# lusinlu/Video-Generation-for-Human-Avatars

Measured on AMD Instinct MI355X. Metric: LTX-2B LoRA train-step samples/sec (latent-tokens/sec = samples/sec x 1792), higher is better.
Workload: dtype bf16; 1 GPU; LTX-Video 2B LoRA(r=16, attn2 q/k/v/out) + caption_projection train step, 49f 512x512 -> latent 7x16x16 (N=1792), 1xMI355X per rank; lora_rank=16, model=LTX-Video-2B (28 layers, D 2048, 32x64 heads), global_batch=8, micro_batch_per_gpu=8, seq_len=1792, text_len=256, grad_accum=16, parallelism=dp1, attn2_padding_blocks=skipped, exact

## Files before the change

### include/ltx_hip.h

```cpp
#ifndef LTX_HIP_H_
#define LTX_HIP_H_

#include <stdint.h>

#ifdef __cplusplus
extern "C" {
#endif

enum {
  LTX_OK = 0,
  LTX_ERR_BAD_ARG = 1000,
  LTX_ERR_UNSUPPORTED = 1001,
};

enum {
  LTX_EPI_STORE = 0,
  LTX_EPI_GELU = 1,
  LTX_EPI_GATED_RESIDUAL = 2,
  LTX_EPI_LORA = 3,
  LTX_EPI_LORA_RESIDUAL = 4,
  LTX_EPI_GELU_BWD = 5,
  LTX_EPI_ACCUM = 6,
  LTX_EPI_LORA_DGRAD_ACCUM = 7,
  LTX_EPI_STORE_ROWDOT = 8,
// ... 4 lines not shown
int ltx_device_info(int* gfx_arch, int* num_cus);

int ltx_patchify_bf16(const void* latents, void* tokens, int64_t B, int64_t C, int64_t F,
                      int64_t H, int64_t W, void* stream);
int ltx_unpatchify_bf16(const void* tokens, void* latents, int64_t B, int64_t C, int64_t F,
                        int64_t H, int64_t W, void* stream);
int ltx_latent_coords(int64_t* coords, int64_t B, int64_t F, int64_t H, int64_t W, void* stream);

int ltx_rf_noise_velocity(const void* tokens, const void* noise, const float* t, void* x_t,
                          void* v_target, int64_t B, int64_t NC, void* stream);
int ltx_rf_noise_velocity_f32(const void* tokens, int tokens_f32, const void* noise, int noise_f32,
                              const float* t, float* x_t, float* v_target, int64_t B, int64_t NC,
                              void* stream);
int ltx_condition_lerp(const void* tokens, const void* ref, const void* pose, void* out,
                       int64_t B, int64_t C, int64_t F, int64_t H, int64_t W, void* stream);
int ltx_rf_prepare_tokens(const void* latents, const void* ref, const void* pose,
                          const void* noise, const float* t, void* x_t, void* model_in,
                          void* v_target, int64_t B, int64_t C, int64_t F, int64_t H, int64_t W,
                          void* stream);

int ltx_rmsnorm_modulate_fwd(const void* x, const void* shift, const void* onep, int64_t ld_mod,
                             void* y, float* rstd, int64_t M, int64_t D, int64_t rows_per_batch,
                             float eps, void* stream);
int ltx_rmsnorm_modulate_bwd(const void* dy, const void* x, const float* rstd, const void* onep,
                             int64_t ld_mod, const void* dres, void* dx, int64_t M, int64_t D,
                             int64_t rows_per_batch, void* stream);
int ltx_rmsnorm_modulate_bwd_gated(const void* dy, const void* x, const float* rstd, const void* onep,
                                   int64_t ld_mod, const void* dres, void* dx, int64_t M, int64_t D,
                                   int64_t rows_per_batch, const void* gate, int64_t ld_gate,
                                   void* gout, void* stream);
int ltx_ada_modulation(const void* sst, const void* tmod, int64_t ld_tmod, int64_t ld_j,
                       void* out, void* onep_out, int64_t B, int64_t P, int64_t D,
                       int64_t scale_mask, void* stream);
int ltx_add_bf16(const void* x, int64_t ldx, const void* y, int64_t ldy, void* out, int64_t ldo, int64_t M,
                 int64_t N, void* stream);
int ltx_gated_residual_bf16(const void* r, int64_t ldr, const void* gate, int64_t ld_gate, const void* y,
                            int64_t ldy, void* out, int64_t ldo, int64_t M, int64_t N, int64_t rows_per_batch,
                            void* stream);
int ltx_gate_mul_bf16(const void* dy, const void* gate, int64_t ld_gate, void* out, int64_t M,
                      int64_t D, int64_t rows_per_batch, void* stream);

int ltx_layernorm_modulate_fwd(const void* x, const void* shift, const void* onep, int64_t ld_mod,
                               void* y, float* mean, float* rstd, int64_t M, int64_t D,
                               int64_t rows_per_batch, float eps, void* stream);
int ltx_layernorm_modulate_bwd(const void* dy, const void* x, const float* mean,
                               const float* rstd, const void* onep, int64_t ld_mod, void* dx,
                               int64_t M, int64_t D, int64_t rows_per_batch, void* stream);

int ltx_rope_pack_bf16(const void* cos, const void* sin, int64_t ld, int64_t rows, int64_t D, uint32_t* cs,
                       void* stream);
int ltx_rope_table(const void* indices_grid, int grid_is_float, int64_t B, int64_t N, int64_t D,
                   const float* omega, float max_pos_t, float max_pos_h, float max_pos_w, uint32_t* cs,
                   void* stream);
int ltx_qk_norm_rope_fwd(const void* q_in, int64_t ldq_in, const void* k_in, int64_t ldk_in,
                         void* q_out, int64_t ldq_out, void* k_out, int64_t ldk_out,
                         const void* q_weight, const void* k_weight, float* rstd_q,
                         float* rstd_k, const uint32_t* rope_cs, int64_t cs_batch_rows, int64_t B,
                         int64_t N, int64_t D, int rope, float eps, void* stream);
int ltx_qk_norm_rope_bwd(const void* dq_in, int64_t ldq_in, int dq_is_f32, const void* dk_in,
                         int64_t ldk_in, int dk_is_f32, const void* q_raw, int64_t ldq_raw,
                         const void* k_raw, int64_t ldk_raw, const void* q_weight,
                         const void* k_weight, const float* rstd_q, const float* rstd_k,
                         void* dq_out, int64_t ldq_out, void* dk_out, int64_t ldk_out,
                         const uint32_t* rope_cs, int64_t cs_batch_rows, int64_t B, int64_t N,
                         int64_t D, int rope, void* stream);
int ltx_qk_norm_fwd_grouped(const void* x, int64_t ldx, int64_t x_gs, void* y, int64_t ldy, int64_t y_gs,
// ... 191 lines not shown
```

### video-generation-for-human-avatars_amd/csrc/elementwise.hip

```cpp
#include <cmath>
#include <cstdlib>
#include <string>

#include "adamw_elem.h"
#include "common.h"
#include "ltx_hip.h"

namespace ltx {

static thread_local std::string g_last_error;
void set_error(const std::string& msg) { g_last_error = msg; }
int fail(int code, const std::string& msg) {
  g_last_error = msg;
  return code;
}

constexpr int TT = 64;
__global__ __launch_bounds__(256) void transpose_kernel(const bf16_t* __restrict__ in, int64_t ld_in,
                                                        int64_t bstride_in, bf16_t* __restrict__ out,
                                                        int64_t ld_out, int64_t bstride_out, int R, int C) {
  __shared__ bf16_t tile[TT][TT + 2];
  const int b = blockIdx.z;
  const int r0 = blockIdx.y * TT, c0 = blockIdx.x * TT;
  const bf16_t* src = in + (int64_t)b * bstride_in;
// ... 160 lines not shown
    if (onep && ((scale_mask >> j) & 1u)) onep[i] = f2bf(1.0f + s);
  }
}

__global__ __launch_bounds__(256) void ada_v8_kernel(const bf16_t* __restrict__ sst, const bf16_t* __restrict__ tmod,
                                                     int64_t ld_tmod, int64_t ld_j, bf16_t* __restrict__ out,
                                                     bf16_t* __restrict__ onep, int B, int P, int D,
                                                     unsigned scale_mask) {
  const int64_t rows = (int64_t)B * P;
  const int D8 = D / 8;
  for (int64_t row = blockIdx.x; row < rows; row += gridDim.x) {
    const int j = (int)(row % P);
    const int64_t b = row / P;
    const bf16_t* tp = tmod + b * ld_tmod + (int64_t)j * ld_j;
    const bf16_t* sp = sst + (int64_t)j * D;
    bf16_t* op = out + row * D;
    const bool sc = onep && ((scale_mask >> j) & 1u);
    for (int c = threadIdx.x; c < D8; c += 256) {
      const u32x4 a = *(const u32x4*)(sp + 8 * c), t = *(const u32x4*)(tp + 8 * c);
      u32x4 o, q;
#pragma unroll
      for (int h = 0; h < 4; ++h) {
        const float s0 = rbf(bf2f((bf16_t)(a[h] & 0xffff)) + bf2f((bf16_t)(t[h] & 0xffff)));
        const float s1 = rbf(bf2f((bf16_t)(a[h] >> 16)) + bf2f((bf16_t)(t[h] >> 16)));
        o[h] = pack2(s0, s1);
        q[h] = pack2(1.0f + s0, 1.0f + s1);
      }
      *(u32x4*)(op + 8 * c) = o;
      if (sc) *(u32x4*)(onep + row * D + 8 * c) = q;
    }
  }
}

__global__ __launch_bounds__(256) void gated_residual_kernel(const bf16_t* r, int64_t ldr,
                                                             const bf16_t* __restrict__ gate, int64_t ldg,
                                                             const bf16_t* __restrict__ y, int64_t ldy, bf16_t* out,
                                                             int64_t ldo, int64_t M, int N, int rpb) {
  const int N8 = N / 8;
  const int64_t total = M * N8;
  for (int64_t i = blockIdx.x * (int64_t)blockDim.x + threadIdx.x; i < total; i += (int64_t)gridDim.x * blockDim.x) {
    const int64_t m = i / N8;
    const int c = (int)(i - m * N8) * 8;
    const u32x4 r4 = *(const u32x4*)(r + m * ldr + c);
    const u32x4 g4 = *(const u32x4*)(gate + (m / rpb) * ldg + c);
    const u32x4 y4 = *(const u32x4*)(y + m * ldy + c);
    u32x4 o;
#pragma unroll
    for (int h = 0; h < 4; ++h) {
      float v[2];
#pragma unroll
      for (int e = 0; e < 2; ++e) {
        const float rv = bf2f((bf16_t)(r4[h] >> (16 * e))), gv = bf2f((bf16_t)(g4[h] >> (16 * e)));
        const float yv = bf2f((bf16_t)(y4[h] >> (16 * e)));
        v[e] = rv + rbf(gv * yv);
      }
      o[h] = pack2(v[0], v[1]);
    }
    *(u32x4*)(out + m * ldo + c) = o;
  }
}

__global__ __launch_bounds__(256) void add_rows_kernel(const bf16_t* x, int64_t ldx, const bf16_t* __restrict__ y,
                                                       int64_t ldy, bf16_t* out, int64_t ldo, int64_t M, int N) {
  const int N8 = N / 8;
  const int64_t total = M * N8;
  for (int64_t i = blockIdx.x * (int64_t)blockDim.x + threadIdx.x; i < total; i += (int64_t)gridDim.x * blockDim.x) {
// ... 272 lines not shown
                          const float* t, void* x_t, void* model_in, void* v_target, int64_t B, int64_t C,
                          int64_t F, int64_t H, int64_t W, void* stream) {
  LTX_CHECK_ARG(latents && ref && pose && noise && t && model_in && v_target, "rf_prepare_tokens: null");
  LTX_CHECK_ARG(B > 0 && C > 0 && F > 0 && H > 0 && W > 0, "rf_prepare_tokens: bad shape");
  const int64_t N = F * H * W;
  dim3 grid((unsigned)((N + TT - 1) / TT), (unsigned)((C + TT - 1) / TT), (unsigned)B);
  hipLaunchKernelGGL(prep_tokens_kernel<0>, grid, dim3(256), 0, (hipStream_t)stream, (const bf16_t*)latents,
                     (const bf16_t*)ref, (const bf16_t*)pose, (const bf16_t*)noise, t, (bf16_t*)x_t,
                     (bf16_t*)model_in, (bf16_t*)v_target, (int)C, (int)F, (int)(H * W));
  LTX_LAUNCH_CHECK();
  return LTX_OK;
}

int ltx_ada_modulation(const void* sst, const void* tmod, int64_t ld_tmod, int64_t ld_j, void* out, void* onep_out,
                       int64_t B, int64_t P, int64_t D, int64_t scale_mask, void* stream) {
  LTX_CHECK_ARG(sst && tmod && out && B > 0 && P > 0 && P <= 32 && D > 0, "ada_modulation: bad args");
  const int64_t total = B * P * D;
  if (D % 8 == 0 && ld_tmod % 8 == 0 && ld_j % 8 == 0 &&
      (((uintptr_t)sst | (uintptr_t)tmod | (uintptr_t)out | (uintptr_t)onep_out) % 16) == 0) {
    const int64_t rows = B * P;
    hipLaunchKernelGGL(ada_v8_kernel, dim3((unsigned)(rows < 16384 ? rows : 16384)), dim3(256), 0,
                       (hipStream_t)stream, (const bf16_t*)sst, (const bf16_t*)tmod, ld_tmod, ld_j, (bf16_t*)out,
                       (bf16_t*)onep_out, (int)B, (int)P, (int)D, (unsigned)scale_mask);
    LTX_LAUNCH_CHECK();
    return LTX_OK;
  }
  hipLaunchKernelGGL(ada_kernel, dim3(grid_for(total)), dim3(256), 0, (hipStream_t)stream, (const bf16_t*)sst,
                     (const bf16_t*)tmod, ld_tmod, ld_j, (bf16_t*)out, (bf16_t*)onep_out, (int)B, (int)P, (int)D,
                     (unsigned)scale_mask);
  LTX_LAUNCH_CHECK();
  return LTX_OK;
}

int ltx_timestep_embedding(const float* t, float scale, void* out, int64_t B, int64_t dim, void* stream) {
  LTX_CHECK_ARG(t && out && B > 0 && dim > 0 && dim % 2 == 0, "timestep_embedding: bad args");
  hipLaunchKernelGGL(timestep_kernel, dim3(grid_for(B * dim)), dim3(256), 0, (hipStream_t)stream, t, scale,
                     (bf16_t*)out, (int)B, (int)dim);
  LTX_LAUNCH_CHECK();
  return LTX_OK;
}

int ltx_add_bf16(const void* x, int64_t ldx, const void* y, int64_t ldy, void* out, int64_t ldo, int64_t M,
                 int64_t N, void* stream) {
  LTX_CHECK_ARG(x && y && out && M > 0 && N > 0 && N % 8 == 0 && ldx % 8 == 0 && ldy % 8 == 0 && ldo % 8 == 0 &&
                    (((uintptr_t)x | (uintptr_t)y | (uintptr_t)out) % 16) == 0,
                "add_bf16: rows must be 16-B aligned, N % 8 == 0");
  hipLaunchKernelGGL(add_rows_kernel, dim3(grid_for(M * N / 8)), dim3(256), 0, (hipStream_t)stream, (const bf16_t*)x,
                     ldx, (const bf16_t*)y, ldy, (bf16_t*)out, ldo, M, (int)N);
  LTX_LAUNCH_CHECK();
  return LTX_OK;
}

int ltx_gated_residual_bf16(const void* r, int64_t ldr, const void* gate, int64_t ld_gate, const void* y,
                            int64_t ldy, void* out, int64_t ldo, int64_t M, int64_t N, int64_t rows_per_batch,
                            void* stream) {
  LTX_CHECK_ARG(r && gate && y && out && M > 0 && N > 0 && N % 8 == 0, "gated_residual: bad args");
  LTX_CHECK_ARG(ldr % 8 == 0 && ld_gate % 8 == 0 && ldy % 8 == 0 && ldo % 8 == 0 &&
                    (((uintptr_t)r | (uintptr_t)gate | (uintptr_t)y | (uintptr_t)out) % 16) == 0,
                "gated_residual: rows must be 16-B aligned");
  const int rpb = (int)(rows_per_batch > 0 ? rows_per_batch : M);
  hipLaunchKernelGGL(gated_residual_kernel, dim3(grid_for(M * N / 8)), dim3(256), 0, (hipStream_t)stream,
                     (const bf16_t*)r, ldr, (const bf16_t*)gate, ld_gate, (const bf16_t*)y, ldy, (bf16_t*)out, ldo,
                     M, (int)N, rpb);
  LTX_LAUNCH_CHECK();
  return LTX_OK;
}
// ... 86 lines not shown
```

### video-generation-for-human-avatars_amd/ltx_amd/_lib.py

```python
import ctypes
import os
import threading

import torch

_HERE = os.path.dirname(os.path.abspath(__file__))
LIB_PATH = os.environ.get("LTX_HIP_LIB", os.path.join(_HERE, "libltxhip.so"))

_i64 = ctypes.c_int64
_i32 = ctypes.c_int
_f32 = ctypes.c_float
_f64 = ctypes.c_double
_p = ctypes.c_void_p

_SIGNATURES = {
    "ltx_abi_version": [],
    "ltx_device_info": [ctypes.POINTER(_i32), ctypes.POINTER(_i32)],
    "ltx_patchify_bf16": [_p, _p, _i64, _i64, _i64, _i64, _i64, _p],
    "ltx_unpatchify_bf16": [_p, _p, _i64, _i64, _i64, _i64, _i64, _p],
    "ltx_latent_coords": [_p, _i64, _i64, _i64, _i64, _p],
    "ltx_rf_noise_velocity": [_p, _p, _p, _p, _p, _i64, _i64, _p],
    "ltx_rf_noise_velocity_f32": [_p, _i32, _p, _i32, _p, _p, _p, _i64, _i64, _p],
    "ltx_condition_lerp": [_p, _p, _p, _p, _i64, _i64, _i64, _i64, _i64, _p],
    "ltx_rf_prepare_tokens": [_p, _p, _p, _p, _p, _p, _p, _p, _i64, _i64, _i64, _i64, _i64, _p],
    "ltx_rmsnorm_modulate_fwd": [_p, _p, _p, _i64, _p, _p, _i64, _i64, _i64, _f32, _p],
    "ltx_rmsnorm_modulate_bwd": [_p, _p, _p, _p, _i64, _p, _p, _i64, _i64, _i64, _p],
    "ltx_rmsnorm_modulate_bwd_gated": [_p, _p, _p, _p, _i64, _p, _p, _i64, _i64, _i64, _p, _i64, _p,
                                       _p],
    "ltx_ada_modulation": [_p, _p, _i64, _i64, _p, _p, _i64, _i64, _i64, _i64, _p],
    "ltx_gate_mul_bf16": [_p, _p, _i64, _p, _i64, _i64, _i64, _p],
    "ltx_layernorm_modulate_fwd": [_p, _p, _p, _i64, _p, _p, _p, _i64, _i64, _i64, _f32, _p],
    "ltx_layernorm_modulate_bwd": [_p, _p, _p, _p, _p, _i64, _p, _i64, _i64, _i64, _p],
    "ltx_rope_table": [_p, _i32, _i64, _i64, _i64, _p, _f32, _f32, _f32, _p, _p],
    "ltx_rope_pack_bf16": [_p, _p, _i64, _i64, _i64, _p, _p],
    "ltx_qk_norm_rope_fwd": [_p, _i64, _p, _i64, _p, _i64, _p, _i64, _p, _p, _p, _p, _p, _i64,
                             _i64, _i64, _i64, _i32, _f32, _p],
    "ltx_qk_norm_rope_bwd": [_p, _i64, _i32, _p, _i64, _i32, _p, _i64, _p, _i64, _p, _p, _p, _p,
                             _p, _i64, _p, _i64, _p, _i64, _i64, _i64, _i64, _i32, _p],
    "ltx_qk_norm_fwd_grouped": [_p, _i64, _i64, _p, _i64, _i64, _p, _i64, _p, _i64, _i64, _i64, _i64,
                                _f32, _p],
    "ltx_qk_norm_bwd_grouped": [_p, _i64, _i64, _p, _i64, _i64, _p, _i64, _p, _i64, _p, _i64, _i64,
                                _i64, _i64, _i64, _p],
    "ltx_attn_fwd": [_p, _i64, _p, _i64, _p, _i64, _p, _i64, _p, _p, _i64, _i64, _i64, _i64, _i64,
                     _i64, _f32, _p],
    "ltx_attn_bwd": [_p, _i64, _p, _i64, _p, _i64, _p, _i64, _p, _i64, _p, _p, _p, _p, _i64, _i32,
                     _p, _i64, _p, _i64, _i64, _i64, _i64, _i64, _i64, _i64, _f32, _p],
    "ltx_attn_reload_switches": [],
    "ltx_attn_bwd_ex": [_p, _i64, _p, _i64, _p, _i64, _p, _i64, _p, _i64, _p, _p, _p, _i32, _p,
                        _i64, _i32, _p, _i64, _p, _i64, _i64, _i64, _i64, _i64, _i64, _i64, _f32,
                        _p],
    "ltx_gemm_bf16_nt": [_p, _i64, _p, _i64, _p, _i64, _i64, _i64, _i64, _i32, _p, _p, _i64, _p,
                         _i64, _p, _i64, _f32, _i64, _i64, _p],
    "ltx_gemm_set_variant": [_i32],
    "ltx_gemm_describe": [_i64, _i64, _i64, _i64, _i32, _i64, _p, _p, _i64],
    "ltx_add_bf16": [_p, _i64, _p, _i64, _p, _i64, _i64, _i64, _p],
    "ltx_gated_residual_bf16": [_p, _i64, _p, _i64, _p, _i64, _p, _i64, _i64, _i64, _i64, _p],
    "ltx_gemm_set_workspace": [_p, _i64],
    "ltx_gemm_set_stream_workspace": [_p, _p, _i64],
    "ltx_gemm_bf16_nt_ext": [_p, _i64, _p, _i64, _p, _i64, _p, _i64, _i64, _p, _i64, _i64, _i64,
                             _i64, _i32, _p, _p, _i64, _p, _i64, _p, _i64, _f32, _i64, _i64, _p],
    "ltx_gemm_bf16_nt_gext": [_p, _i64, _p, _i64, _p, _i64, _p, _i64, _i64, _i64, _i64, _p, _i64,
                              _i64, _i64, _i64, _i32, _p, _p, _i64, _p, _i64, _p, _i64, _f32, _i64,
# ... 130 lines not shown
```

### video-generation-for-human-avatars_amd/ltx_amd/ops.py

```python
import ctypes
import functools
import os

import torch

from . import _lib
from ._lib import EPI, call

BF16 = torch.bfloat16
F32 = torch.float32


def _p(t):
    return None if t is None else ctypes.c_void_p(t.data_ptr())


def _s():
    return _lib.stream_ptr()


def _rows(t, name):
    if t.dim() != 2 or t.stride(1) != 1:
        raise ValueError(f"{name}: expected a 2-D row-major view, got shape {tuple(t.shape)} "
                         f"strides {t.stride()}")
# ... 69 lines not shown
            raise _lib.LtxHipError(f"{n}: tensor is not on a ROCm device (no CPU fallback)")
    if noise.shape != tokens.shape:
        raise ValueError("rf_noise_velocity_f32: tokens and noise shapes differ")
    B = tokens.shape[0]
    t = t.to(device=tokens.device, dtype=F32).reshape(-1)
    if t.numel() != B:
        raise ValueError(f"rf_noise_velocity_f32: {t.numel()} timesteps for batch {B}")
    x_t = torch.empty(tokens.shape, dtype=F32, device=tokens.device) if want_x else None
    v = torch.empty(tokens.shape, dtype=F32, device=tokens.device) if want_v else None
    call("ltx_rf_noise_velocity_f32", _p(tokens.contiguous()), 1 if tokens.dtype == F32 else 0,
         _p(noise.contiguous()), 1 if noise.dtype == F32 else 0, _p(t.contiguous()), _p(x_t), _p(v),
         B, tokens[0].numel(), _s())
    return x_t, v


def condition_lerp(tokens, ref, pose, out=None):
    _need(tokens, BF16, "tokens")
    B, C, F, H, W = pose.shape
    tokens = tokens.contiguous()
    out = torch.empty(tokens.shape, dtype=BF16, device=tokens.device) if out is None else out
    call("ltx_condition_lerp", _p(tokens), _p(ref.contiguous()),
         _p(pose.contiguous()), _p(out), B, C, F, H, W, _s())
    return out


def ada_modulation(sst, tmod, scale_mask, broadcast=False):
    P, D = sst.shape
    B = tmod.shape[0]
    ld = _rows(tmod, "tmod")
    out = torch.empty(B, P, D, dtype=BF16, device=sst.device)
    onep = torch.empty(B, P, D, dtype=BF16, device=sst.device)
    call("ltx_ada_modulation", _p(sst.contiguous()), _p(tmod), ld, 0 if broadcast else D, _p(out),
         _p(onep), B, P, D, scale_mask, _s())
    return out, onep


def gate_mul(dy, gate, rows_per_batch):
    M, D = dy.shape
    dy = dy.contiguous()
    out = torch.empty(M, D, dtype=BF16, device=dy.device)
    call("ltx_gate_mul_bf16", _p(dy), _p(gate), _rows(gate, "gate"), _p(out), M, D, rows_per_batch,
         _s())
    return out


def _dense(t, name):
    if not t.is_contiguous():
        raise ValueError(f"{name}: expected a dense [M, D] tensor")
    return t


def rmsnorm_modulate_fwd(x, shift, onep, ld_mod, rows_per_batch, eps, out=None):
    M, D = _dense(x, "x").shape
    y = torch.empty(M, D, dtype=BF16, device=x.device) if out is None else out
    rstd = torch.empty(M, dtype=F32, device=x.device)
    call("ltx_rmsnorm_modulate_fwd", _p(x), _p(shift), _p(onep), ld_mod, _p(y), _p(rstd), M, D,
         rows_per_batch, eps, _s())
    return y, rstd


def rmsnorm_modulate_bwd(dy, x, rstd, onep, ld_mod, rows_per_batch, dres=None, out=None,
                         gate=None):
    M, D = _dense(x, "x").shape
    _dense(dy, "dy")
    dx = torch.empty(M, D, dtype=BF16, device=x.device) if out is None else out
    if gate is None:
# ... 917 lines not shown
```

### video-generation-for-human-avatars_amd/ltx_amd/transformer3d.py

```python
import glob
import json
import math
import os
from dataclasses import dataclass
from enum import Enum, auto
from pathlib import Path
from typing import Any, Dict, List, NamedTuple, Optional

import torch
from torch import nn

from . import _lib, ops
from .patchifier import SymmetricPatchifier

OURS_TRANSFORMER_CONFIG = {
    "_class_name": "Transformer3DModel",
    "activation_fn": "gelu-approximate",
    "attention_bias": True,
    "attention_head_dim": 64,
    "attention_type": "default",
    "caption_channels": 4096,
    "cross_attention_dim": 2048,
    "double_self_attention": False,
    "dropout": 0.0,
# ... 683 lines not shown
    lora, lora1, loraf = _lora_params(blk), _lora_params1(blk), _lora_params_ff(blk)
    r, s = (0, 1.0) if lora is None else (lora[0].r, lora[0].scaling)
    r1, s1 = (0, 1.0) if lora1 is None else (lora1[0].r, lora1[0].scaling)
    rf, sf = (0, 1.0) if loraf is None else (loraf[0].r, loraf[0].scaling)
    return _BlockLora(lora, lora1, loraf, r, s, r1, s1, rf, sf, lora is not None and lora[0].use_dora)


def _block_ab(blk):
    groups = (_lora_params(blk), _lora_params1(blk), _lora_params_ff(blk))
    return [t for g in groups if g is not None for m in g for t in _ab(m)]


class _Saved(NamedTuple):
    base: tuple
    attn2: tuple
    full: tuple
    attn1: tuple
    ff: tuple
    x2: Optional[torch.Tensor]


def _pack_saved(base, attn2=(), full=(), attn1=(), ff=(), x2=None):
    x2 = () if x2 is None else (x2,)
    return ((*base, *attn2, *full, *attn1, *ff, *x2),
            (len(base), len(attn2), len(full), len(attn1), len(ff), len(x2)))


def _unpack_saved(flat, layout):
    groups, i = [], 0
    for n in layout:
        groups.append(flat[i:i + n])
        i += n
    return _Saved(*groups[:5], groups[5][0] if groups[5] else None)


class _BlockFn(torch.autograd.Function):

    @staticmethod
    def forward(ctx, blk, sh, keep, skip, h, enc2, mods, onep, *lora_ab):
        B, N, L, H, d, D = sh.B, sh.N, sh.L, sh.H, sh.d, sh.D
        M = B * N
        rpm = sh.rpm
        if skip is not None and keep:
            raise NotImplementedError("skip-layer masks are an inference (forward-only) feature")
        W = blk.weights()
        a1, a2 = blk.attn1, blk.attn2
        ldm = mods.stride(0)
        ad = _block_lora(blk)
        ab2, ab1, abf = ad.split(lora_ab)
        lora, lora1, loraf = ad.attn2, ad.attn1, ad.ff
        full = sh.full and keep
        if lora_ab and full:
            raise NotImplementedError("train_mode='full' trains the base weights without LoRA")
        dp = sh.block_drop(blk) if keep else None
        x1, rstd1 = ops.rmsnorm_modulate_fwd(h, mods[:, 0], onep[:, 1], ldm, rpm, blk.norm_eps)
        if lora1 is not None:
            u1, su1 = _qkv_lora_down(x1, lora1, ab1, ad.r1, dp)
            ext_w, grouped, _ = _qkv_ext(blk, lora1[0], lora1[1], lora1[2])
            qkv = ops.gemm(x1, W["qkv_w"], bias=W["qkv_b"], ext=(su1, ext_w),
                           ext_group=(D, ops.lora_k2(ad.r1)) if grouped else None)
            del su1
        else:
            qkv = ops.gemm(x1, W["qkv_w"], bias=W["qkv_b"])
        strat = skip[1] if skip is not None else None
        keep_x1 = full or (lora1 is not None and keep)
        if strat is not SkipLayerStrategy.AttentionSkip and not keep_x1:
# ... 147 lines not shown
            if not full:
                dk2b = dv2b = None
        else:
            dq2, dk2, dv2 = ops.attn_bwd(q2, k2, v2, o2, do2, lse2, B, H, d, a2.scale,
                                         key_bias=sh.enc_bias, dk=dk2_keep, dv=dkv[:, D:], delta=delta2)
        del do2
        dq2raw, _ = ops.qk_norm_rope_bwd(dq2, q2raw, a2.q_norm.weight, rq2, B=B, N=N)
        if dk2_keep is None:
            dk2raw, _ = ops.qk_norm_rope_bwd(dk2, k2raw, a2.k_norm.weight, rk2, B=sh.Bt, N=L,
                                             dq_out=dkv[:, :D])
        else:
            dk2raw = None
        if full:
            ops.qk_norm_wgrad_into(dq2, q2raw, rq2, _pgrad(a2.q_norm.weight), B=B, N=N)
            ops.wgrad_into(_pgrad(a2.to_q.weight), dq2raw, h1)
            ops.colsum_into(_pgrad(a2.to_q.bias), dq2raw)
            if dk2b is not None:
                krep, erep, rrep = k2raw.repeat(B, 1), enc2.repeat(B, 1), rk2.repeat(B)
                dk2raw_b, _ = ops.qk_norm_rope_bwd(dk2b, krep, a2.k_norm.weight, rrep, B=B, N=L)
                ops.qk_norm_wgrad_into(dk2b, krep, rrep, _pgrad(a2.k_norm.weight), B=B, N=L)
                ops.wgrad_into(_pgrad(a2.to_k.weight), dk2raw_b, erep)
                ops.colsum_into(_pgrad(a2.to_k.bias), dk2raw_b)
                ops.wgrad_into(_pgrad(a2.to_v.weight), dv2b, erep)
                ops.colsum_into(_pgrad(a2.to_v.bias), dv2b)
                del krep, erep, rrep, dk2raw_b, dk2b, dv2b
            else:
                ops.qk_norm_wgrad_into(dk2, k2raw, rk2, _pgrad(a2.k_norm.weight), B=sh.Bt, N=L)
                ops.wgrad_into(_pgrad(a2.to_k.weight), dk2raw, enc2)
                ops.colsum_into(_pgrad(a2.to_k.bias), dk2raw)
                ops.wgrad_into(_pgrad(a2.to_v.weight), dv2, enc2)
                ops.colsum_into(_pgrad(a2.to_v.bias), dv2)
        del dq2, dk2
        denc = None
        d_y1 = torch.empty_like(dh2)
        gated = dict(aux1=mods[:, 2], aux2=d_y1, rows_per_batch=rpm)
        dh1 = _lora_dgrad(dq2raw, W["q2_wT"], lq, Aq, Bq, u_q, h1, r, s, dp, 4, epi=gated, dora=dora,
                          epilogue="accum", aux0=dh2)
        if lora is not None and dp is not None:
            d_y1 = ops.gate_mul(dh1, mods[:, 2], rpm)
        if dora:
            ops.dora_mag_grad(dq2raw, q2raw, _lin(lq)[1], _dora_m(lq), _grad_buf(lq, "m"))
        if tx is None and lora is not None:
            denc = _text_kv_lora_backward(blk, dkv, (dk2raw, dv2), (k2raw, v2), (u_k, u_v), (lk, lv),
                                          (Ak, Bk, Av, Bv), enc2, W["kv2_wT"], r, s, dp, dora)
        elif tx is None:
            denc = ops.gemm(dkv, W["kv2_wT"])
        del dq2raw, dk2raw, dv2, dh2, dkv
        fused1 = _DELTA_FUSED and not (lora1 is not None and dp is not None)
        delta1 = torch.empty(B, H, N, dtype=torch.float32, device=h.device) if fused1 else None
        rd = dict(epilogue="store_rowdot", aux0=o1, aux1=delta1, rank=d, rows_per_batch=N) \
            if fused1 else {}
        do1 = _lora_dgrad(d_y1, W["out1_wT"], lo1, Ao1, Bo1, u_o1, o1, r1, s1, dp, 3, epi=rd)
        if full:
            ops.colsum_into(dmods[:, 2], dh1, y1, mode=1, rows_per_group=rpm, sum_groups=False,
                            accumulate=False)
            lin = a1.to_out[0]
            ops.wgrad_into(_pgrad(lin.weight), d_y1, o1)
            ops.colsum_into(_pgrad(lin.bias), d_y1)
        del d_y1
        M = B * N
        dqkv = torch.empty(M, 3 * D, dtype=torch.bfloat16, device=h.device)
        dq1, dk1, _ = ops.attn_bwd(qk[:, :D], qk[:, D:], qkv[:, 2 * D:], o1, do1, lse1, B, H, d,
                                   a1.scale, dv=dqkv[:, 2 * D:], delta=delta1)
        del do1
        ops.qk_norm_rope_bwd(dq1, qkv[:, :D], a1.q_norm.weight, rq1, dk1, qkv[:, D:2 * D],
                             a1.k_norm.weight, rk1, sh.rope, dq_out=dqkv[:, :D],
                             dk_out=dqkv[:, D:2 * D])
        if full:
            ops.qk_norm_wgrad_into(dq1, qkv[:, :D], rq1, _pgrad(a1.q_norm.weight), dk1,
                                   qkv[:, D:2 * D], rk1, _pgrad(a1.k_norm.weight), rope=sh.rope)
            dwqkv = ops.wgrad(dqkv, x1)
            for i, lin in enumerate((a1.to_q, a1.to_k, a1.to_v)):
                ops.add_into(_pgrad(lin.weight), dwqkv[i * D:(i + 1) * D])
                ops.colsum_into(_pgrad(lin.bias), dqkv[:, i * D:(i + 1) * D])
            del dwqkv
        del dq1, dk1
        dh = None
        if lora1 is not None and dp is not None:
            w1 = torch.empty(M, 3 * r1, dtype=torch.float32, device=h.device)
            for g in range(3):
                xd = _drop_x(x1, dp, g)
                _lora_backward(dqkv[:, g * D:(g + 1) * D], u1[:, g * r1:(g + 1) * r1], lora1[g], ab1[2 * g + 1],
                               xd, r1, s1, w_out=w1[:, g * r1:(g + 1) * r1], da_alpha=dp[2])
                del xd
        elif lora1 is not None:
            sw1 = _qkv_lora_backward(dqkv, u1, lora1, ab1, x1, r1, s1)
        if ctx.needs_input_grad[4] or full:
            if lora1 is not None and dp is not None:
                dx1 = ops.gemm(dqkv, W["qkv_wT"])
                _masked_add(dx1, w1, [ab1[0], ab1[2], ab1[4]], dp, (0, 1, 2))
            elif lora1 is not None:
                dx1 = ops.gemm(dqkv, W["qkv_wT"], ext=(sw1, _qkv_ext(blk, lora1[0], lora1[1], lora1[2])[2]))
            else:
                dx1 = ops.gemm(dqkv, W["qkv_wT"])
            g_prev = None if full else sh.ffgate.get(id(blk))
            if g_prev is not None:
                dh, d_ffo_prev = ops.rmsnorm_modulate_bwd(dx1, h, rstd1, onep[:, 1], ldm, rpm,
                                                          dres=dh1, gate=g_prev)
                sh.ffo_pre = (dh, d_ffo_prev)
                del d_ffo_prev
            else:
                dh = ops.rmsnorm_modulate_bwd(dx1, h, rstd1, onep[:, 1], ldm, rpm, dres=dh1)
            if full:
                ops.colsum_into(dmods[:, 0], dx1, rows_per_group=rpm, sum_groups=False,
                                accumulate=False)
                ops.colsum_into(dmods[:, 1], dx1, h, rstd1, mode=2, rows_per_group=rpm,
                                sum_groups=False, accumulate=False)
        dm = dmods if full else None
        done = None if tx is None else tx.token_params[tx.index[id(blk)]]
        for cb in getattr(blk, "_grad_ready_hooks", ()):
            cb(blk, done)
        return (None, None, None, None, dh, denc, dm, None, *(None,) * ad.n_ab)


class _CaptionProjFn(torch.autograd.Function):

    @staticmethod
    def forward(ctx, enc, w1, b1, w2, b2):
        pre = torch.empty(enc.shape[0], w1.shape[0], dtype=torch.int16, device=enc.device)
        act = ops.gemm(enc, w1, bias=b1, epilogue="gelu", aux0=pre)
        out = ops.gemm(act, w2, bias=b2)
        ctx.save_for_backward(enc, pre, act, w2)
        return out

    @staticmethod
    def backward(ctx, dout):
        enc, pre, act, w2 = ctx.saved_tensors
        dout = dout.contiguous()
        dw2 = ops.wgrad(dout, act)
        db2 = ops.colsum(dout)
        dpre = ops.gemm(dout, ops.transpose(w2), epilogue="gelu_bwd", aux0=pre)
        dw1 = ops.wgrad(dpre, enc)
        db1 = ops.colsum(dpre)
        return None, dw1, db1, dw2, db2


def _text_kv(blk, sh, enc2, lora_ab, dp=None):
    a2 = blk.attn2
    W = blk.weights()
    D = sh.D
    if lora_ab:
        lora = _lora_params(blk)
        _, _, Ak, _, Av, _, _, _ = lora_ab
        K2 = ops.lora_k2(lora[1].r)
        su = torch.empty(enc2.shape[0], 2 * K2, dtype=torch.bfloat16, device=enc2.device)
# ... 333 lines not shown
                nk = k
                for a, b in TRANSFORMER_KEYS_RENAME_DICT.items():
                    nk = nk.replace(a, b)
                renamed[nk] = v
            state = renamed
        elif path.is_file() and str(path).endswith(".safetensors"):
            state = {}
            with safe_open(str(path), framework="pt", device="cpu") as f:
                metadata = f.metadata()
                for k in f.keys():
                    state[k] = f.get_tensor(k)
            config = json.loads(metadata["config"])["transformer"]
        else:
            raise FileNotFoundError(str(path))
        with torch.device("meta"):
            model = cls.from_config(config)
        model.load_state_dict(state, assign=True, strict=True)
        patchifier = kwargs.get("patchifier")
        if patchifier is not None:
            model.patchifier = patchifier
        return model

    def _text_knorm_weights(self, blocks, D):
        knws = [b.attn2.k_norm.weight for b in blocks]
        if not all(w is not None and w.dtype == torch.bfloat16 and w.numel() == D for w in knws):
            return None
        key = tuple((w.data_ptr(), w._version) for w in knws)
        c = getattr(self, "_knw_cache", None)
        if c is None or c[0] != key:
            c = (key, torch.stack([w.detach() for w in knws]).contiguous())
            self._knw_cache = c
        return c[1]

    def _text_structure(self):
        blocks = list(self.transformer_blocks)
        if not (_TEXT_BATCH and blocks):
            return None
        lins = [_lora_params(b) for b in blocks]
        if any(l is None for l in lins):
            return None
        if any(m.use_dora for l in lins for m in l):
            return None
        key = tuple((id(l[1]), id(l[2]), _base(l[1])._parameters["weight"].requires_grad,
                     _base(l[2])._parameters["weight"].requires_grad,
                     id(b._modules["attn1"]._modules["to_q"]),
                     id(b._modules["ff"]._modules["net"]._modules["2"])) for l, b in zip(lins, blocks))
        c = getattr(self, "_tx_struct", None)
        if c is not None and c[0] == key:
            return c[1]
        r, sc = lins[0][1].r, lins[0][1].scaling
        ok = (2 * blocks[0].attn2.inner_dim) % 256 == 0 and all(
            l[1].r == r and l[2].r == r and l[1].scaling == sc and l[2].scaling == sc
            and not k[2] and not k[3] for l, k in zip(lins, key))
        st = None
        if ok:
            block_params = [list(_ab(l[1]) + _ab(l[2])) for l in lins]
            text_ids = {id(p) for ps in block_params for p in ps}
            st = {"blocks": blocks, "lins": lins, "adapters": [m for l in lins for m in (l[1], l[2])],
                  "index": {id(b): i for i, b in enumerate(blocks)}, "block_params": block_params,
                  "token_params": [[p for p in b.parameters() if id(p) not in text_ids]
                                   for b in blocks],
                  "text_ids": text_ids, "r": r, "s": sc, "D": blocks[0].attn2.inner_dim}
        self._tx_struct = (key, st)
        return st

    def _lora_dropout_plan(self):
# ... 175 lines not shown
                skip_layer_strategy, Enum) else SkipLayerStrategy[str(skip_layer_strategy)]
            if strat is SkipLayerStrategy.Residual:
                strat = None
        blocks = list(self.transformer_blocks)
        if _TEXT_STREAM and not keep and h.is_cuda and len(blocks) > 1:
            side = _side_stream(h.device)
            main = torch.cuda.current_stream()
            sh.text_pre = {}

            def prep(j):
                bj = blocks[j]
                with torch.no_grad():
                    bj.weights()
                    lj = _lora_params(bj)
                    if lj is not None:
                        _kv_ext(bj, lj[1], lj[2])
                ready = torch.cuda.Event()
                ready.record(main)
                with torch.no_grad(), torch.cuda.stream(side):
                    side.wait_event(ready)
                    vals = _text_kv(bj, sh, enc2, [t for m in lj or () for t in _ab(m)])
                    ev = torch.cuda.Event()
                    ev.record(side)
                for t in vals:
                    if t is not None:
                        t.record_stream(main)
                sh.text_pre[id(bj)] = (vals, ev)
            prep(0)
        else:
            prep = None
        fuse_gate = keep and not ckpt and not full and strat is None and \
            os.environ.get("LTX_FFGATE_FUSED", "1") != "0"
        prev_gate = None
        for i, blk in enumerate(self.transformer_blocks):
            if prep is not None and i + 1 < len(blocks):
                prep(i + 1)
            skip = None if strat is None else (skip_layer_mask[i].to(dt).contiguous(), strat)
            if full:
                mods, onep = _AdaModFn.apply(blk.scale_shift_table, tmod, (1 << 1) | (1 << 4),
                                             False)
            else:
                with torch.no_grad():
                    mods, onep = ops.ada_modulation(blk.scale_shift_table, tmod,
                                                    (1 << 1) | (1 << 4))
            ab = _block_ab(blk)
            if fuse_gate:
                if prev_gate is not None:
                    sh.ffgate[id(blk)] = prev_gate
                prev_gate = mods[:, 5]
            if ckpt:
                h = torch.utils.checkpoint.checkpoint(
                    lambda *a, _b=blk, _s=skip: _BlockFn.apply(_b, sh, True, _s, *a),
                    h, enc2, mods, onep, *ab, use_reentrant=False)
            else:
                h = _BlockFn.apply(blk, sh, keep, skip, h, enc2, mods, onep, *ab)
        if full:
            hmod, honep = _AdaModFn.apply(self.scale_shift_table, emb, 1 << 1, True)
        else:
            with torch.no_grad():
                hmod, honep = ops.ada_modulation(self.scale_shift_table, emb, 1 << 1,
                                                 broadcast=True)
        out = _HeadFn.apply(h, hmod, honep, self.proj_out.weight, self.proj_out.bias, sh.rpm, 1e-6)
        return out.view(B, N, self.out_channels)

    def _adaln(self, timestep):
        mult = float(self.timestep_scale_multiplier or 1.0)
        ad = self.adaln_single
        te = ops.timestep_embedding(timestep.reshape(-1).float().contiguous(), mult)
        e1 = ops.gemm(te, ad.emb.timestep_embedder.linear_1.weight,
                      bias=ad.emb.timestep_embedder.linear_1.bias)
        emb = ops.gemm(ops.silu(e1), ad.emb.timestep_embedder.linear_2.weight,
                       bias=ad.emb.timestep_embedder.linear_2.bias)
        tmod = ops.gemm(ops.silu(emb), ad.linear.weight, bias=ad.linear.bias)
# ... 2 lines not shown
```

Measured before the change: 70.03 samples/s.

## Batch per-block ada modulation into one launch and truncate backward at first needed layer

Adds an ada_blocks kernel that computes the modulation tensors for all transformer blocks in a single launch from a cached stacked scale_shift_table, replacing 28 separate per-block launches. Separately, a backward 'frontier' path stops a block's backward after the attn2 LoRA weight gradients when the input gradient is not needed and attn1 has no LoRA. That skips the q2 dgrad GEMM and the rest of that block's backward (attn1, FF, norms). This trades a small cache and a stacked copy for fewer launches, and relies on the needs_input_grad check being correct for the first block.

```diff
diff --git a/include/ltx_hip.h b/include/ltx_hip.h
--- a/include/ltx_hip.h
+++ b/include/ltx_hip.h
@@ -60,6 +60,9 @@
 int ltx_ada_modulation(const void* sst, const void* tmod, int64_t ld_tmod, int64_t ld_j,
                        void* out, void* onep_out, int64_t B, int64_t P, int64_t D,
                        int64_t scale_mask, void* stream);
+int ltx_ada_blocks(const void* sst, int64_t ld_l, int64_t ld_p, const void* tmod, int64_t ld_tmod,
+                   int64_t ld_j, void* out, void* onep_out, int64_t Lyr, int64_t B, int64_t P,
+                   int64_t D, int64_t scale_mask, void* stream);
 int ltx_add_bf16(const void* x, int64_t ldx, const void* y, int64_t ldy, void* out, int64_t ldo, int64_t M,
                  int64_t N, void* stream);
 int ltx_gated_residual_bf16(const void* r, int64_t ldr, const void* gate, int64_t ld_gate, const void* y,
diff --git a/video-generation-for-human-avatars_amd/csrc/elementwise.hip b/video-generation-for-human-avatars_amd/csrc/elementwise.hip
--- a/video-generation-for-human-avatars_amd/csrc/elementwise.hip
+++ b/video-generation-for-human-avatars_amd/csrc/elementwise.hip
@@ -216,6 +216,46 @@
   }
 }
 
+template <bool V8>
+__global__ __launch_bounds__(256) void ada_blocks_kernel(const bf16_t* __restrict__ sst, int64_t ld_l, int64_t ld_p,
+                                                         const bf16_t* __restrict__ tmod, int64_t ld_tmod,
+                                                         int64_t ld_j, bf16_t* __restrict__ out,
+                                                         bf16_t* __restrict__ onep, int Lyr, int B, int P, int D,
+                                                         unsigned scale_mask) {
+  const int64_t rows = (int64_t)Lyr * B * P;
+  for (int64_t row = blockIdx.x; row < rows; row += gridDim.x) {
+    const int j = (int)(row % P);
+    const int64_t lb = row / P;
+    const int64_t b = lb % B, l = lb / B;
+    const bf16_t* tp = tmod + b * ld_tmod + (int64_t)j * ld_j;
+    const bf16_t* sp = sst + l * ld_l + (int64_t)j * ld_p;
+    bf16_t* op = out + row * D;
+    bf16_t* qp = onep + row * D;
+    const bool sc = (scale_mask >> j) & 1u;
+    if constexpr (V8) {
+      for (int c = threadIdx.x; c < D / 8; c += 256) {
+        const u32x4 a = *(const u32x4*)(sp + 8 * c), t = *(const u32x4*)(tp + 8 * c);
+        u32x4 o, q;
+#pragma unroll
+        for (int h = 0; h < 4; ++h) {
+          const float s0 = rbf(bf2f((bf16_t)(a[h] & 0xffff)) + bf2f((bf16_t)(t[h] & 0xffff)));
+          const float s1 = rbf(bf2f((bf16_t)(a[h] >> 16)) + bf2f((bf16_t)(t[h] >> 16)));
+          o[h] = pack2(s0, s1);
+          q[h] = pack2(1.0f + s0, 1.0f + s1);
+        }
+        *(u32x4*)(op + 8 * c) = o;
+        if (sc) *(u32x4*)(qp + 8 * c) = q;
+      }
+    } else {
+      for (int c = threadIdx.x; c < D; c += 256) {
+        const float s = rbf(bf2f(sp[c]) + bf2f(tp[c]));
+        op[c] = f2bf(s);
+        if (sc) qp[c] = f2bf(1.0f + s);
+      }
+    }
+  }
+}
+
 __global__ __launch_bounds__(256) void gated_residual_kernel(const bf16_t* r, int64_t ldr,
                                                              const bf16_t* __restrict__ gate, int64_t ldg,
                                                              const bf16_t* __restrict__ y, int64_t ldy, bf16_t* out,
@@ -554,6 +594,28 @@
   return LTX_OK;
 }
 
+int ltx_ada_blocks(const void* sst, int64_t ld_l, int64_t ld_p, const void* tmod, int64_t ld_tmod, int64_t ld_j,
+                   void* out, void* onep_out, int64_t Lyr, int64_t B, int64_t P, int64_t D, int64_t scale_mask,
+                   void* stream) {
+  LTX_CHECK_ARG(sst && tmod && out && onep_out && Lyr > 0 && B > 0 && P > 0 && P <= 32 && D > 0 && ld_p >= D &&
+                    ld_l >= 0 && ld_tmod >= 0 && ld_j >= 0 && Lyr * B * P < ((int64_t)1 << 31),
+                "ada_blocks: bad args");
+  const int64_t rows = Lyr * B * P;
+  const dim3 grid((unsigned)(rows < 16384 ? rows : 16384)), blk(256);
+  const bool v8 = D % 8 == 0 && ld_l % 8 == 0 && ld_p % 8 == 0 && ld_tmod % 8 == 0 && ld_j % 8 == 0 &&
+                  (((uintptr_t)sst | (uintptr_t)tmod | (uintptr_t)out | (uintptr_t)onep_out) % 16) == 0;
+  if (v8)
+    hipLaunchKernelGGL(ada_blocks_kernel<true>, grid, blk, 0, (hipStream_t)stream, (const bf16_t*)sst, ld_l, ld_p,
+                       (const bf16_t*)tmod, ld_tmod, ld_j, (bf16_t*)out, (bf16_t*)onep_out, (int)Lyr, (int)B, (int)P,
+                       (int)D, (unsigned)scale_mask);
+  else
+    hipLaunchKernelGGL(ada_blocks_kernel<false>, grid, blk, 0, (hipStream_t)stream, (const bf16_t*)sst, ld_l, ld_p,
+                       (const bf16_t*)tmod, ld_tmod, ld_j, (bf16_t*)out, (bf16_t*)onep_out, (int)Lyr, (int)B, (int)P,
+                       (int)D, (unsigned)scale_mask);
+  LTX_LAUNCH_CHECK();
+  return LTX_OK;
+}
+
 int ltx_timestep_embedding(const float* t, float scale, void* out, int64_t B, int64_t dim, void* stream) {
   LTX_CHECK_ARG(t && out && B > 0 && dim > 0 && dim % 2 == 0, "timestep_embedding: bad args");
   hipLaunchKernelGGL(timestep_kernel, dim3(grid_for(B * dim)), dim3(256), 0, (hipStream_t)stream, t, scale,
diff --git a/video-generation-for-human-avatars_amd/ltx_amd/_lib.py b/video-generation-for-human-avatars_amd/ltx_amd/_lib.py
--- a/video-generation-for-human-avatars_amd/ltx_amd/_lib.py
+++ b/video-generation-for-human-avatars_amd/ltx_amd/_lib.py
@@ -28,6 +28,7 @@
     "ltx_rmsnorm_modulate_bwd_gated": [_p, _p, _p, _p, _i64, _p, _p, _i64, _i64, _i64, _p, _i64, _p,
                                        _p],
     "ltx_ada_modulation": [_p, _p, _i64, _i64, _p, _p, _i64, _i64, _i64, _i64, _p],
+    "ltx_ada_blocks": [_p, _i64, _i64, _p, _i64, _i64, _p, _p, _i64, _i64, _i64, _i64, _i64, _p],
     "ltx_gate_mul_bf16": [_p, _p, _i64, _p, _i64, _i64, _i64, _p],
     "ltx_layernorm_modulate_fwd": [_p, _p, _p, _i64, _p, _p, _p, _i64, _i64, _i64, _f32, _p],
     "ltx_layernorm_modulate_bwd": [_p, _p, _p, _p, _p, _i64, _p, _i64, _i64, _i64, _p],
diff --git a/video-generation-for-human-avatars_amd/ltx_amd/ops.py b/video-generation-for-human-avatars_amd/ltx_amd/ops.py
--- a/video-generation-for-human-avatars_amd/ltx_amd/ops.py
+++ b/video-generation-for-human-avatars_amd/ltx_amd/ops.py
@@ -125,6 +125,21 @@
     onep = torch.empty(B, P, D, dtype=BF16, device=sst.device)
     call("ltx_ada_modulation", _p(sst.contiguous()), _p(tmod), ld, 0 if broadcast else D, _p(out),
          _p(onep), B, P, D, scale_mask, _s())
+    return out, onep
+
+
+def ada_blocks(sst, tmod, scale_mask):
+    _need(sst, BF16, "ada_blocks sst")
+    _need(tmod, BF16, "ada_blocks tmod")
+    Lyr, P, D = sst.shape
+    if sst.stride(2) != 1 or tmod.shape[1] != P * D:
+        raise ValueError(f"ada_blocks: sst strides {sst.stride()} / tmod shape {tuple(tmod.shape)}")
+    B = tmod.shape[0]
+    ld = _rows(tmod, "tmod")
+    out = torch.empty(Lyr, B, P, D, dtype=BF16, device=sst.device)
+    onep = torch.empty(Lyr, B, P, D, dtype=BF16, device=sst.device)
+    call("ltx_ada_blocks", _p(sst), sst.stride(0), sst.stride(1), _p(tmod), ld, D, _p(out), _p(onep),
+         Lyr, B, P, D, scale_mask, _s())
     return out, onep
 
 
diff --git a/video-generation-for-human-avatars_amd/ltx_amd/transformer3d.py b/video-generation-for-human-avatars_amd/ltx_amd/transformer3d.py
--- a/video-generation-for-human-avatars_amd/ltx_amd/transformer3d.py
+++ b/video-generation-for-human-avatars_amd/ltx_amd/transformer3d.py
@@ -739,6 +739,16 @@
         groups.append(flat[i:i + n])
         i += n
     return _Saved(*groups[:5], groups[5][0] if groups[5] else None)
+
+
+_BWD_FRONTIER = os.environ.get("LTX_BWD_FRONTIER", "1") != "0"
+
+
+def _block_backward_done(blk, tx, ad, dh, denc, dm):
+    done = None if tx is None else tx.token_params[tx.index[id(blk)]]
+    for cb in getattr(blk, "_grad_ready_hooks", ()):
+        cb(blk, done)
+    return (None, None, None, None, dh, denc, dm, None, *(None,) * ad.n_ab)
 
 
 class _BlockFn(torch.autograd.Function):
@@ -952,12 +962,19 @@
                 ops.colsum_into(_pgrad(a2.to_v.bias), dv2)
         del dq2, dk2
         denc = None
-        d_y1 = torch.empty_like(dh2)
-        gated = dict(aux1=mods[:, 2], aux2=d_y1, rows_per_batch=rpm)
-        dh1 = _lora_dgrad(dq2raw, W["q2_wT"], lq, Aq, Bq, u_q, h1, r, s, dp, 4, epi=gated, dora=dora,
-                          epilogue="accum", aux0=dh2)
-        if lora is not None and dp is not None:
-            d_y1 = ops.gate_mul(dh1, mods[:, 2], rpm)
+        frontier = _BWD_FRONTIER and not ctx.needs_input_grad[4] and not full and lora1 is None
+        if frontier:
+            if lq is not None:
+                xq = h1 if dp is None else _drop_x(h1, dp, 4)
+                _lora_backward(dq2raw, u_q, lq, Bq, xq, r, s, da_alpha=1.0 if dp is None else dp[2], dora=dora)
+                del xq
+        else:
+            d_y1 = torch.empty_like(dh2)
+            gated = dict(aux1=mods[:, 2], aux2=d_y1, rows_per_batch=rpm)
+            dh1 = _lora_dgrad(dq2raw, W["q2_wT"], lq, Aq, Bq, u_q, h1, r, s, dp, 4, epi=gated, dora=dora,
+                              epilogue="accum", aux0=dh2)
+            if lora is not None and dp is not None:
+                d_y1 = ops.gate_mul(dh1, mods[:, 2], rpm)
         if dora:
             ops.dora_mag_grad(dq2raw, q2raw, _lin(lq)[1], _dora_m(lq), _grad_buf(lq, "m"))
         if tx is None and lora is not None:
@@ -966,6 +983,8 @@
         elif tx is None:
             denc = ops.gemm(dkv, W["kv2_wT"])
         del dq2raw, dk2raw, dv2, dh2, dkv
+        if frontier:
+            return _block_backward_done(blk, tx, ad, None, denc, None)
         fused1 = _DELTA_FUSED and not (lora1 is not None and dp is not None)
         delta1 = torch.empty(B, H, N, dtype=torch.float32, device=h.device) if fused1 else None
         rd = dict(epilogue="store_rowdot", aux0=o1, aux1=delta1, rank=d, rows_per_batch=N) \
@@ -1026,11 +1045,7 @@
                                 accumulate=False)
                 ops.colsum_into(dmods[:, 1], dx1, h, rstd1, mode=2, rows_per_group=rpm,
                                 sum_groups=False, accumulate=False)
-        dm = dmods if full else None
-        done = None if tx is None else tx.token_params[tx.index[id(blk)]]
-        for cb in getattr(blk, "_grad_ready_hooks", ()):
-            cb(blk, done)
-        return (None, None, None, None, dh, denc, dm, None, *(None,) * ad.n_ab)
+        return _block_backward_done(blk, tx, ad, dh, denc, dmods if full else None)
 
 
 class _CaptionProjFn(torch.autograd.Function):
@@ -1430,6 +1445,18 @@
             self._knw_cache = c
         return c[1]
 
+    @torch.no_grad()
+    def _sst_stack(self):
+        ts = [b._parameters["scale_shift_table"] for b in self.transformer_blocks]
+        key = (tuple((t.data_ptr(), t._version) for t in ts),
+               ops.weight_generation() if any(t.requires_grad for t in ts) else 0)
+        c = getattr(self, "_sst_cache", None)
+        if c is None or c[0] != key:
+            self._sst_cache = None
+            c = (key, torch.stack([t.detach() for t in ts]).contiguous())
+            self._sst_cache = c
+        return c[1]
+
     def _text_structure(self):
         blocks = list(self.transformer_blocks)
         if not (_TEXT_BATCH and blocks):
@@ -1671,6 +1698,10 @@
         fuse_gate = keep and not ckpt and not full and strat is None and \
             os.environ.get("LTX_FFGATE_FUSED", "1") != "0"
         prev_gate = None
+        mods_all = onep_all = None
+        if blocks and not full and not per_token:
+            with torch.no_grad():
+                mods_all, onep_all = ops.ada_blocks(self._sst_stack(), tmod, (1 << 1) | (1 << 4))
         for i, blk in enumerate(self.transformer_blocks):
             if prep is not None and i + 1 < len(blocks):
                 prep(i + 1)
@@ -1678,6 +1709,8 @@
             if full:
                 mods, onep = _AdaModFn.apply(blk.scale_shift_table, tmod, (1 << 1) | (1 << 4),
                                              False)
+            elif mods_all is not None:
+                mods, onep = mods_all[i], onep_all[i]
             else:
                 with torch.no_grad():
                     mods, onep = ops.ada_modulation(blk.scale_shift_table, tmod,
```

Result: no change. 70.70 samples/s, median of 6 (+1.0%).
